# adityaX1412/Experiment-YOLO

Hardware: AMD Instinct MI355X
Metric: images/sec (train) DEAL-YOLO-N 640x640 bs=64/GPU (higher is better)
Workload: dtype f16; 1 GPU; DEAL-YOLO-N (yolov8n-ASF-P2P2.yaml) train step 640x640, per-GPU batch 64, fwd+TAL/WIOU+NWD/DFL/BCE loss+bwd+SGD+EMA, BASELINE.json configs[1]; loss_mode=wiou+nwd, settle_steps=18, capture_retries=0, global_batch=64, parallelism=dp1, hipgraph=True

## Files before the change

experiment-yolo_amd/csrc/bn_act.hip:

```cpp
#include <cstdlib>
#include "common.h"
#include "dealyolo_hip.h"

struct BnFinArgs {
  const float* part[3];
  int nparts[3];
  float pweight[3];
  const float* gamma;
  const float* beta;
  float* running_mean;
  float* running_var;
  float* coef;
  int C;
  float count, eps, momentum;
  int update_running;
  int ldp;
  long long* nbt;
};

__global__ __launch_bounds__(256) void bn_finalize_kernel(BnFinArgs a) {
  const int c = blockIdx.x, tid = threadIdx.x;
  double s1 = 0.0, s2 = 0.0;
  for (int k = 0; k < 3; ++k) {
    if (!a.part[k]) continue;
    double t1 = 0.0, t2 = 0.0;
    for (int i = tid; i < a.nparts[k]; i += 256) {
      t1 += a.part[k][((size_t)i * 2 + 0) * a.ldp + c];
      t2 += a.part[k][((size_t)i * 2 + 1) * a.ldp + c];
    }
    s1 += t1 * a.pweight[k];
    s2 += t2 * a.pweight[k];
  }
  __shared__ double r1[256], r2[256];
  r1[tid] = s1;
  r2[tid] = s2;
  __syncthreads();
  for (int o = 128; o > 0; o >>= 1) {
    if (tid < o) {
      r1[tid] += r1[tid + o];
      r2[tid] += r2[tid + o];
    }
    __syncthreads();
  }
  if (tid == 0) {
    const double mean = r1[0] / a.count;
    double var = r2[0] / a.count - mean * mean;
    if (var < 0.0) var = 0.0;
    const float invstd = (float)(1.0 / sqrt(var + (double)a.eps));
    const float sc = a.gamma[c] * invstd;
    a.coef[0 * a.C + c] = sc;
    a.coef[1 * a.C + c] = a.beta[c] - (float)mean * sc;
    a.coef[2 * a.C + c] = (float)mean;
    a.coef[3 * a.C + c] = invstd;
    if (a.update_running) {
      const double unbiased = a.count > 1.f ? var * a.count / (a.count - 1.0) : var;
      a.running_mean[c] = (1.f - a.momentum) * a.running_mean[c] + a.momentum * (float)mean;
      a.running_var[c] = (1.f - a.momentum) * a.running_var[c] + a.momentum * (float)unbiased;
      if (a.nbt && c == 0) *a.nbt += 1;
    }
  }
}

extern "C" int dy_bn_finalize(const float* p0, int n0, float w0, const float* p1, int n1, float w1, const float* p2,
                              int n2, float w2, const float* gamma, const float* beta, float* running_mean,
                              float* running_var, float* coef, int C, float count, float eps, float momentum,
                              int update_running, hipStream_t stream) {
  BnFinArgs a{{p0, p1, p2}, {n0, n1, n2}, {w0, w1, w2}, gamma, beta, running_mean, running_var, coef, C, count, eps,
              momentum, update_running, C, nullptr};
  hipLaunchKernelGGL(bn_finalize_kernel, dim3(C), dim3(256), 0, stream, a);
  DY_CHECK_LAUNCH();
  return DY_OK;
}
extern "C" int dy_bn_finalize_ld(const float* part, int nparts, int ldp, const float* gamma, const float* beta, float* running_mean,
                                 float* running_var, float* coef, int C, float count, float eps, float momentum, int update_running,
                                 long long* num_batches_tracked, hipStream_t stream) {
  if (C < 1 || ldp < C || nparts < 1 || !part || !gamma || !beta || !coef || (update_running && (!running_mean || !running_var))) return DY_ERR_ARG;
  BnFinArgs a{{part, nullptr, nullptr}, {nparts, 0, 0}, {1.f, 0.f, 0.f}, gamma, beta, running_mean, running_var, coef, C, count, eps,
              momentum, update_running, ldp, update_running ? num_batches_tracked : nullptr};
  hipLaunchKernelGGL(bn_finalize_kernel, dim3(C), dim3(256), 0, stream, a);
  DY_CHECK_LAUNCH();
  return DY_OK;
}

__global__ void bn_eval_coef_kernel(const float* g, const float* b, const float* rm, const float* rv, float* coef, int C,
                                    float eps) {
  const int c = blockIdx.x * blockDim.x + threadIdx.x;
  if (c >= C) return;
  const float invstd = 1.f / sqrtf(rv[c] + eps), sc = g[c] * invstd;
  coef[c] = sc;
  coef[C + c] = b[c] - rm[c] * sc;
  coef[2 * C + c] = rm[c];
  coef[3 * C + c] = invstd;
}
extern "C" int dy_bn_eval_coef(const float* gamma, const float* beta, const float* rm, const float* rv, float* coef,
                               int C, float eps, hipStream_t stream) {
  hipLaunchKernelGGL(bn_eval_coef_kernel, dim3(cdiv(C, 64)), dim3(64), 0, stream, gamma, beta, rm, rv, coef, C, eps);
  DY_CHECK_LAUNCH();
  return DY_OK;
}

#define DY_ACT_DISPATCH(KERNEL, grid, stream, args)                                                        \
  do {                                                                                                     \
    if (act == DY_ACT_SILU) hipLaunchKernelGGL(KERNEL<DY_ACT_SILU>, grid, dim3(256), 0, stream, args);      \
    else if (act == DY_ACT_LEAKY) hipLaunchKernelGGL(KERNEL<DY_ACT_LEAKY>, grid, dim3(256), 0, stream, args); \
    else hipLaunchKernelGGL(KERNEL<DY_ACT_NONE>, grid, dim3(256), 0, stream, args);                         \
  } while (0)

static __device__ __forceinline__ float act_fwd(float z, int act) {
  if (act == DY_ACT_SILU) return silu_f(z);
  if (act == DY_ACT_LEAKY) return z > 0.f ? z : 0.1f * z;
  return z;
}
static __device__ __forceinline__ float act_grad(float z, int act) {
  if (act == DY_ACT_SILU) {
    const float s = sigmoid_f(z);
    return s * (1.f + z * (1.f - s));
  }
  if (act == DY_ACT_LEAKY) return z > 0.f ? 1.f : 0.1f;
  return 1.f;
}

struct ApplyArgs {
  const f16* x;
  const f16* res;
  f16* y;
  const float* coef;
  int ldx, ldr, ldy, C, act;
  long npix;
  int rev;
  f16* y2 = nullptr;
  int ldy2 = 0, csplit = 1 << 30;
};

struct BnAccFwd {
  const double* acc;
  const float* gamma;
  const float* beta;
  float* running_mean;
  float* running_var;
  float* coef_out;
  float count, eps, momentum;
};

template <int ACT, bool ACC, bool FAST = false>
static __device__ __forceinline__ void bn_act_apply_body(const ApplyArgs& a, const BnAccFwd& b, const int bx, const int nb) {
  const int cpp = a.C >> 3, rows = 256 / cpp;
  const int part = threadIdx.x % cpp, row = threadIdx.x / cpp, c0 = part * 8;
  extern __shared__ float s_coef[];
  if (ACC) {
    for (int c = threadIdx.x; c < a.C; c += 256) {
      double s1 = 0.0, s2 = 0.0;
#pragma unroll
      for (int k = 0; k < DY_BN_COPIES; ++k) {
        s1 += b.acc[(size_t)(k * 2 + 0) * a.C + c];
        s2 += b.acc[(size_t)(k * 2 + 1) * a.C + c];
      }
      const double mean = s1 / b.count;
      double var = s2 / b.count - mean * mean;
      if (var < 0.0) var = 0.0;
      const float invstd = (float)(1.0 / sqrt(var + (double)b.eps));
      const float scl = b.gamma[c] * invstd, shf = b.beta[c] - (float)mean * scl;
      s_coef[c] = scl;
      s_coef[a.C + c] = shf;
      if (bx == 0) {
        b.coef_out[c] = scl;
        b.coef_out[a.C + c] = shf;
        b.coef_out[2 * a.C + c] = (float)mean;
        b.coef_out[3 * a.C + c] = invstd;
        const double unbiased = b.count > 1.f ? var * b.count / (b.count - 1.0) : var;
        b.running_mean[c] = (1.f - b.momentum) * b.running_mean[c] + b.momentum * (float)mean;
        b.running_var[c] = (1.f - b.momentum) * b.running_var[c] + b.momentum * (float)unbiased;
      }
    }
    __syncthreads();
  }
  if (row >= rows) return;
  float sc[8], sh[8];
#pragma unroll
  for (int j = 0; j < 8; ++j) {
    sc[j] = ACC ? s_coef[c0 + j] : a.coef[c0 + j];
    sh[j] = ACC ? s_coef[a.C + c0 + j] : a.coef[a.C + c0 + j];
  }
  auto at = [&](long p) { return a.rev ? a.npix - 1 - p : p; };
  f16* const yb = c0 < a.csplit ? a.y + c0 : a.y2 + (c0 - a.csplit);
  const int ly = c0 < a.csplit ? a.ldy : a.ldy2;
  auto one = [&](long pix, const half8& xv) {
    pix = at(pix);
    half8 rv;
    if (a.res) rv = *reinterpret_cast<const half8*>(a.res + pix * a.ldr + c0);
    half8 out;
    if (FAST) {
#pragma unroll
      for (int j = 0; j < 8; j += 2) {
        f32x2 z = act_fwd2_fast<ACT>(__builtin_elementwise_fma((f32x2){(float)xv[j], (float)xv[j + 1]}, (f32x2){sc[j], sc[j + 1]},
                                                               (f32x2){sh[j], sh[j + 1]}));
        if (a.res) z += (f32x2){(float)rv[j], (float)rv[j + 1]};
        const half2_ oh = __builtin_convertvector(z, half2_);
        out[j] = oh[0];
        out[j + 1] = oh[1];
      }
    } else {
#pragma unroll
      for (int j = 0; j < 8; ++j) {
        float z = act_fwd_t<ACT>((float)xv[j] * sc[j] + sh[j]);
        if (a.res) z += (float)rv[j];
        out[j] = (f16)z;
      }
    }
    *reinterpret_cast<half8*>(yb + pix * ly) = out;
  };
  const long step = (long)nb * rows;
  long pix = (long)bx * rows + row;
  for (; pix + step < a.npix; pix += 2 * step) {
    const half8 x0 = *reinterpret_cast<const half8*>(a.x + at(pix) * a.ldx + c0);
    const half8 x1 = *reinterpret_cast<const half8*>(a.x + at(pix + step) * a.ldx + c0);
    one(pix, x0);
    one(pix + step, x1);
  }
  if (pix < a.npix) one(pix, *reinterpret_cast<const half8*>(a.x + at(pix) * a.ldx + c0));
}

template <int ACT, bool ACC, bool FAST = false>
__global__ __launch_bounds__(256) void bn_act_apply_kernel(ApplyArgs a, BnAccFwd b) {
  bn_act_apply_body<ACT, ACC, FAST>(a, b, (int)blockIdx.x, (int)gridDim.x);
}
#define DY_BN_GROUP_MAX 8
struct ApplyGroup {
  int n;
  int nblk[DY_BN_GROUP_MAX];
  ApplyArgs a[DY_BN_GROUP_MAX];
  BnAccFwd b[DY_BN_GROUP_MAX];
};
__global__ __launch_bounds__(256) void bn_act_apply_group_kernel(ApplyGroup g) {
  const int e = blockIdx.y;
  if ((int)blockIdx.x >= g.nblk[e]) return;
  bn_act_apply_body<DY_ACT_SILU, true, true>(g.a[e], g.b[e], (int)blockIdx.x, g.nblk[e]);
}

static inline int ew_reverse() {
  static const int rev = getenv("DY_EW_REVERSE") ? atoi(getenv("DY_EW_REVERSE")) : 4;
  return rev;
}

static long ew_cap(const char* env, long dflt) {
  static struct { const char* name; long cap; } seen[8];
  static int n = 0;
  for (int i = 0; i < n; ++i)
    if (seen[i].name == env) return seen[i].cap;
  const char* e = getenv(env);
  const long cap = e ? atol(e) : dflt;
  if (n < 8) seen[n++] = {env, cap};
  return cap;
}
static inline int ew_blocks(long npix, int C, const char* env, long dflt) {
  const int rows = 256 / (C >> 3);
  long blocks = (npix + (long)rows * 4 - 1) / ((long)rows * 4);
  const long cap = ew_cap(env, dflt);
  if (blocks > cap) blocks = cap;
  if (blocks < 1) blocks = 1;
  return (int)blocks;
}

extern "C" int dy_bn_act_apply(const void* x, int ldx, const void* res, int ldr, void* y, int ldy, const float* coef,
                               long npix, int C, int act, hipStream_t stream) {
  if ((C & 7) || (ldx & 7) || (ldy & 7) || (res && (ldr & 7))) return DY_ERR_ALIGN;
  if ((C >> 3) > 256) return DY_ERR_ARG;
  const int rev = ew_reverse();
  ApplyArgs a{(const f16*)x, (const f16*)res, (f16*)y, coef, ldx, ldr, ldy, C, act, npix, rev & 1};
  const BnAccFwd b{};
  const dim3 grid(ew_blocks(npix, C, "DY_EW_BLOCKS_APPLY", 8192));
  if (act == DY_ACT_SILU) hipLaunchKernelGGL((bn_act_apply_kernel<DY_ACT_SILU, false>), grid, dim3(256), 0, stream, a, b);
  else if (act == DY_ACT_LEAKY) hipLaunchKernelGGL((bn_act_apply_kernel<DY_ACT_LEAKY, false>), grid, dim3(256), 0, stream, a, b);
  else hipLaunchKernelGGL((bn_act_apply_kernel<DY_ACT_NONE, false>), grid, dim3(256), 0, stream, a, b);
  DY_CHECK_LAUNCH();
  return DY_OK;
}

extern "C" int dy_bn_act_apply_acc(const void* x, int ldx, const void* res, int ldr, void* y, int ldy, const double* acc,
                                   const float* gamma, const float* beta, float* running_mean, float* running_var,
                                   float* coef, long npix, int C, int act, float count, float eps, float momentum,
                                   hipStream_t stream) {
  if ((C & 7) || (ldx & 7) || (ldy & 7) || (res && (ldr & 7))) return DY_ERR_ALIGN;
  if ((C >> 3) > 256 || !acc || !gamma || !beta || !running_mean || !running_var || !coef) return DY_ERR_ARG;
  const int rev = ew_reverse();
  ApplyArgs a{(const f16*)x, (const f16*)res, (f16*)y, nullptr, ldx, ldr, ldy, C, act, npix, rev & 1};
  const BnAccFwd b{acc, gamma, beta, running_mean, running_var, coef, count, eps, momentum};
  const dim3 grid(ew_blocks(npix, C, "DY_EW_BLOCKS_APPLY_ACC", 8192));
  const size_t lds = 2 * (size_t)C * sizeof(float);
  static const bool fast = !getenv("DY_SILU_FAST") || atoi(getenv("DY_SILU_FAST"));
  if (act == DY_ACT_SILU && fast) hipLaunchKernelGGL((bn_act_apply_kernel<DY_ACT_SILU, true, true>), grid, dim3(256), lds, stream, a, b);
  else if (act == DY_ACT_SILU) hipLaunchKernelGGL((bn_act_apply_kernel<DY_ACT_SILU, true>), grid, dim3(256), lds, stream, a, b);
  else if (act == DY_ACT_LEAKY) hipLaunchKernelGGL((bn_act_apply_kernel<DY_ACT_LEAKY, true>), grid, dim3(256), lds, stream, a, b);
  else hipLaunchKernelGGL((bn_act_apply_kernel<DY_ACT_NONE, true>), grid, dim3(256), lds, stream, a, b);
  DY_CHECK_LAUNCH();
  return DY_OK;
}

extern "C" int dy_bn_act_apply_acc_split(const void* x, int ldx, void* y, int ldy, void* y2, int ldy2, int csplit, const double* acc,
                                         const float* gamma, const float* beta, float* running_mean, float* running_var, float* coef,
                                         long npix, int C, int act, float count, float eps, float momentum, hipStream_t stream) {
  if ((C & 7) || (ldx & 7) || (ldy & 7) || (ldy2 & 7) || (csplit & 7) || csplit <= 0 || csplit >= C || !y2) return DY_ERR_ALIGN;
  if ((C >> 3) > 256 || !acc || !gamma || !beta || !running_mean || !running_var || !coef) return DY_ERR_ARG;
  const int rev = ew_reverse();
  ApplyArgs a{(const f16*)x, nullptr, (f16*)y, nullptr, ldx, 0, ldy, C, act, npix, rev & 1};
  a.y2 = (f16*)y2; a.ldy2 = ldy2; a.csplit = csplit;
  const BnAccFwd b{acc, gamma, beta, running_mean, running_var, coef, count, eps, momentum};
  const dim3 grid(ew_blocks(npix, C, "DY_EW_BLOCKS_APPLY_ACC", 8192));
  const size_t lds = 2 * (size_t)C * sizeof(float);
  if (act == DY_ACT_SILU) hipLaunchKernelGGL((bn_act_apply_kernel<DY_ACT_SILU, true, true>), grid, dim3(256), lds, stream, a, b);
  else if (act == DY_ACT_LEAKY) hipLaunchKernelGGL((bn_act_apply_kernel<DY_ACT_LEAKY, true>), grid, dim3(256), lds, stream, a, b);
  else hipLaunchKernelGGL((bn_act_apply_kernel<DY_ACT_NONE, true>), grid, dim3(256), lds, stream, a, b);
  DY_CHECK_LAUNCH();
  return DY_OK;
}

extern "C" int dy_bn_group_max(void) { return DY_BN_GROUP_MAX; }
extern "C" int dy_bn_act_apply_acc_group(int n, const void* const* x, const int* ldx, void* const* y, const int* ldy, const double* const* acc,
                                         const float* const* gamma, const float* const* beta, float* const* running_mean,
                                         float* const* running_var, float* const* coef, const long* npix, const int* C, const float* count,
                                         const float* eps, const float* momentum, hipStream_t stream) {
  if (n < 1 || n > DY_BN_GROUP_MAX) return DY_ERR_ARG;
  ApplyGroup g{};
  g.n = n;
  int gx = 1, cmax = 0;
  const int rev = ew_reverse();
  for (int e = 0; e < n; ++e) {
    if ((C[e] & 7) || (ldx[e] & 7) || (ldy[e] & 7)) return DY_ERR_ALIGN;
    if ((C[e] >> 3) > 256 || !acc[e] || !gamma[e] || !beta[e] || !running_mean[e] || !running_var[e] || !coef[e]) return DY_ERR_ARG;
    g.a[e] = ApplyArgs{(const f16*)x[e], nullptr, (f16*)y[e], nullptr, ldx[e], 0, ldy[e], C[e], DY_ACT_SILU, npix[e], rev & 1};
    g.b[e] = BnAccFwd{acc[e], gamma[e], beta[e], running_mean[e], running_var[e], coef[e], count[e], eps[e], momentum[e]};
    g.nblk[e] = ew_blocks(npix[e], C[e], "DY_EW_BLOCKS_APPLY_ACC", 8192);
    gx = g.nblk[e] > gx ? g.nblk[e] : gx;
    cmax = C[e] > cmax ? C[e] : cmax;
  }
  hipLaunchKernelGGL(bn_act_apply_group_kernel, dim3(gx, n), dim3(256), 2 * (size_t)cmax * sizeof(float), stream, g);
  DY_CHECK_LAUNCH();
  return DY_OK;
}

struct BwdRedArgs {
  const f16* dy;
  const f16* x;
  const float* coef;
  float* partials;
  int lddy, ldx, C, act;
  long npix;
  int rev;
  double* acc;
  f16* rg;
  int ldrg, rg_acc;
  const f16* dy2 = nullptr;
  int lddy2 = 0, csplit = 1 << 30;
};

template <int ACT, bool RES = false>
static __device__ __forceinline__ void bn_act_bwd_reduce_body(const BwdRedArgs& a, const int bx, const int nb) {
  const int cpp = a.C >> 3, rows = 256 / cpp, tid = threadIdx.x;
  const int part = tid % cpp, row = tid / cpp, c0 = part * 8;
  f32x2 sg[4], sgx[4], sc[4], sh[4];
#pragma unroll
  for (int j = 0; j < 4; ++j) {
    sg[j] = sgx[j] = (f32x2){0.f, 0.f};
    sc[j] = (f32x2){a.coef[c0 + 2 * j], a.coef[c0 + 2 * j + 1]};
    sh[j] = (f32x2){a.coef[a.C + c0 + 2 * j], a.coef[a.C + c0 + 2 * j + 1]};
  }
  if (row < rows) {
    const long step = (long)nb * rows;
    long pix = (long)bx * rows + row;
    auto at = [&](long p) { return a.rev ? a.npix - 1 - p : p; };
    const f16* const dyb = c0 < a.csplit ? a.dy + c0 : a.dy2 + (c0 - a.csplit);
    const int ldd = c0 < a.csplit ? a.lddy : a.lddy2;
    auto pair = [](const half8& v, int j) { return (f32x2){(float)v[2 * j], (float)v[2 * j + 1]}; };
    auto pass_on = [&](long p, const half8& dv) {
      f16* dst = a.rg + at(p) * a.ldrg + c0;
      half8 o = dv;
      if (a.rg_acc) {
        const half8 old = *reinterpret_cast<const half8*>(dst);
#pragma unroll
        for (int j = 0; j < 8; ++j) o[j] = (f16)((float)old[j] + (float)dv[j]);
      }
      *reinterpret_cast<half8*>(dst) = o;
    };
    for (; pix + step < a.npix; pix += 2 * step) {
      const half8 dv0 = *reinterpret_cast<const half8*>(dyb + at(pix) * ldd);
      const half8 xv0 = *reinterpret_cast<const half8*>(a.x + at(pix) * a.ldx + c0);
      const half8 dv1 = *reinterpret_cast<const half8*>(dyb + at(pix + step) * ldd);
      const half8 xv1 = *reinterpret_cast<const half8*>(a.x + at(pix + step) * a.ldx + c0);
      if (RES) {
        pass_on(pix, dv0);
        pass_on(pix + step, dv1);
      }
#pragma unroll
      for (int j = 0; j < 4; ++j) {
        const f32x2 x0 = pair(xv0, j), x1 = pair(xv1, j);
        const f32x2 g0 = pair(dv0, j) * act_grad2<ACT>(__builtin_elementwise_fma(x0, sc[j], sh[j]));
        const f32x2 g1 = pair(dv1, j) * act_grad2<ACT>(__builtin_elementwise_fma(x1, sc[j], sh[j]));
        sg[j] += g0 + g1;
        sgx[j] += __builtin_elementwise_fma(g0, x0, g1 * x1);
      }
    }
    if (pix < a.npix) {
      const half8 dv = *reinterpret_cast<const half8*>(dyb + at(pix) * ldd);
      const half8 xv = *reinterpret_cast<const half8*>(a.x + at(pix) * a.ldx + c0);
      if (RES) pass_on(pix, dv);
#pragma unroll
      for (int j = 0; j < 4; ++j) {
        const f32x2 x = pair(xv, j);
        const f32x2 g = pair(dv, j) * act_grad2<ACT>(__builtin_elementwise_fma(x, sc[j], sh[j]));
        sg[j] += g;
        sgx[j] += g * x;
      }
    }
#pragma unroll
    for (int j = 0; j < 4; ++j)
#pragma unroll
      for (int k = 0; k < 2; ++k)
        sgx[j][k] = (sgx[j][k] - a.coef[2 * a.C + c0 + 2 * j + k] * sg[j][k]) * a.coef[3 * a.C + c0 + 2 * j + k];
  }
  __shared__ float red[2][256][8 + 1];
#pragma unroll
  for (int j = 0; j < 8; ++j) {
    red[0][tid][j] = sg[j >> 1][j & 1];
    red[1][tid][j] = sgx[j >> 1][j & 1];
  }
  __syncthreads();
  for (int i = tid; i < 2 * a.C; i += 256) {
    const int which = i / a.C, c = i - which * a.C, pp = c >> 3, j = c & 7;
    float s = 0.f;
    for (int r = 0; r < rows; ++r) s += red[which][r * cpp + pp][j];
    if (a.acc) unsafeAtomicAdd(&a.acc[((size_t)(bx % DY_BN_COPIES) * 2 + which) * a.C + c], (double)s);
    else a.partials[((size_t)bx * 2 + which) * a.C + c] = s;
  }
}

template <int ACT, bool RES = false>
__global__ __launch_bounds__(256) void bn_act_bwd_reduce_kernel(BwdRedArgs a) {
  bn_act_bwd_reduce_body<ACT, RES>(a, (int)blockIdx.x, (int)gridDim.x);
}
struct BwdRedGroup {
  int n;
  int nblk[DY_BN_GROUP_MAX];
  BwdRedArgs a[DY_BN_GROUP_MAX];
};
__global__ __launch_bounds__(256) void bn_act_bwd_reduce_group_kernel(BwdRedGroup g) {
  const int e = blockIdx.y;
  if ((int)blockIdx.x >= g.nblk[e]) return;
  bn_act_bwd_reduce_body<DY_ACT_SILU, false>(g.a[e], (int)blockIdx.x, g.nblk[e]);
}

extern "C" int dy_bn_act_bwd_reduce(const void* dy, int lddy, const void* x, int ldx, const float* coef,
                                    float* partials, int max_partials, long npix, int C, int act, int* nparts,
                                    hipStream_t stream) {
  if ((C & 7) || C > 2048 || (ldx & 7) || (lddy & 7)) return DY_ERR_ALIGN;
  const int cpp = C >> 3;
  if (cpp > 256) return DY_ERR_ARG;
  const int rows = 256 / cpp;
  long blocks = (npix + (long)rows * 8 - 1) / ((long)rows * 8);
  if (blocks > max_partials) blocks = max_partials;
  static const long bcap = getenv("DY_EW_BLOCKS_BRED") ? atol(getenv("DY_EW_BLOCKS_BRED")) : 1024;
  if (blocks > bcap) blocks = bcap;
  if (blocks < 1) blocks = 1;
  if (nparts) *nparts = (int)blocks;
  const int rev = ew_reverse();
  BwdRedArgs a{(const f16*)dy, (const f16*)x, coef, partials, lddy, ldx, C, act, npix, (rev >> 2) & 1, nullptr, nullptr, 0, 0};
  DY_ACT_DISPATCH(bn_act_bwd_reduce_kernel, dim3((int)blocks), stream, a);
  DY_CHECK_LAUNCH();
  return DY_OK;
}

extern "C" int dy_bn_act_bwd_reduce_acc(const void* dy, int lddy, const void* x, int ldx, const float* coef, double* acc,
                                        long npix, int C, int act, void* res_grad, int ldrg, int res_accumulate, hipStream_t stream) {
  if ((C & 7) || C > 2048 || (ldx & 7) || (lddy & 7) || (res_grad && ((ldrg & 7) || ((uintptr_t)res_grad & 15)))) return DY_ERR_ALIGN;
  const int cpp = C >> 3;
  if (cpp > 256 || !acc) return DY_ERR_ARG;
  const int rows = 256 / cpp;
  long blocks = (npix + (long)rows * 8 - 1) / ((long)rows * 8);
  static const long bcap = getenv("DY_EW_BLOCKS_BRED") ? atol(getenv("DY_EW_BLOCKS_BRED")) : 1024;
  if (blocks > bcap) blocks = bcap;
  if (blocks < 1) blocks = 1;
  const int rev = ew_reverse();
  BwdRedArgs a{(const f16*)dy, (const f16*)x, coef, nullptr, lddy, ldx, C, act, npix, (rev >> 2) & 1, acc, (f16*)res_grad, ldrg, res_accumulate};
  if (res_grad && act == DY_ACT_SILU) hipLaunchKernelGGL((bn_act_bwd_reduce_kernel<DY_ACT_SILU, true>), dim3((int)blocks), dim3(256), 0, stream, a);
  else if (res_grad && act == DY_ACT_LEAKY) hipLaunchKernelGGL((bn_act_bwd_reduce_kernel<DY_ACT_LEAKY, true>), dim3((int)blocks), dim3(256), 0, stream, a);
  else if (res_grad) hipLaunchKernelGGL((bn_act_bwd_reduce_kernel<DY_ACT_NONE, true>), dim3((int)blocks), dim3(256), 0, stream, a);
  else DY_ACT_DISPATCH(bn_act_bwd_reduce_kernel, dim3((int)blocks), stream, a);
  DY_CHECK_LAUNCH();
  return DY_OK;
}

extern "C" int dy_bn_act_bwd_reduce_acc_split(const void* dy, int lddy, const void* dy2, int lddy2, int csplit, const void* x, int ldx,
                                              const float* coef, double* acc, long npix, int C, int act, hipStream_t stream) {
  if ((C & 7) || C > 2048 || (ldx & 7) || (lddy & 7) || (lddy2 & 7) || (csplit & 7) || csplit <= 0 || csplit >= C || !dy2) return DY_ERR_ALIGN;
  const int cpp = C >> 3;
  if (cpp > 256 || !acc) return DY_ERR_ARG;
  const int rows = 256 / cpp;
  long blocks = (npix + (long)rows * 8 - 1) / ((long)rows * 8);
  static const long bcap = getenv("DY_EW_BLOCKS_BRED") ? atol(getenv("DY_EW_BLOCKS_BRED")) : 1024;
  if (blocks > bcap) blocks = bcap;
  if (blocks < 1) blocks = 1;
  const int rev = ew_reverse();
  BwdRedArgs a{(const f16*)dy, (const f16*)x, coef, nullptr, lddy, ldx, C, act, npix, (rev >> 2) & 1, acc, nullptr, 0, 0};
  a.dy2 = (const f16*)dy2; a.lddy2 = lddy2; a.csplit = csplit;
  DY_ACT_DISPATCH(bn_act_bwd_reduce_kernel, dim3((int)blocks), stream, a);
  DY_CHECK_LAUNCH();
  return DY_OK;
}

extern "C" int dy_bn_act_bwd_reduce_acc_group(int n, const void* const* dy, const int* lddy, const void* const* x, const int* ldx,
                                              const float* const* coef, double* const* acc, const long* npix, const int* C, hipStream_t stream) {
  if (n < 1 || n > DY_BN_GROUP_MAX) return DY_ERR_ARG;
  BwdRedGroup g{};
  g.n = n;
  int gx = 1;
  const int rev = ew_reverse();
  static const long bcap = getenv("DY_EW_BLOCKS_BRED") ? atol(getenv("DY_EW_BLOCKS_BRED")) : 1024;
  for (int e = 0; e < n; ++e) {
    if ((C[e] & 7) || C[e] > 2048 || (ldx[e] & 7) || (lddy[e] & 7)) return DY_ERR_ALIGN;
    const int cpp = C[e] >> 3;
    if (cpp > 256 || !acc[e] || !dy[e] || !x[e] || !coef[e]) return DY_ERR_ARG;
    const int rows = 256 / cpp;
    long blocks = (npix[e] + (long)rows * 8 - 1) / ((long)rows * 8);
    if (blocks > bcap) blocks = bcap;
    if (blocks < 1) blocks = 1;
    g.a[e] = BwdRedArgs{(const f16*)dy[e], (const f16*)x[e], coef[e], nullptr, lddy[e], ldx[e], C[e], DY_ACT_SILU, npix[e], (rev >> 2) & 1, acc[e],
                        nullptr, 0, 0};
    g.nblk[e] = (int)blocks;
    gx = g.nblk[e] > gx ? g.nblk[e] : gx;
  }
  hipLaunchKernelGGL(bn_act_bwd_reduce_group_kernel, dim3(gx, n), dim3(256), 0, stream, g);
  DY_CHECK_LAUNCH();
  return DY_OK;
}

struct BwdRedRowsArgs {
  const f16* dy;
  const f16* x;
  const float* coef;
  double* acc;
  const int* flag;
  int lddy, ldx, C, A, a0, hw, B;
};
template <int ACT>
__global__ __launch_bounds__(256) void bn_act_bwd_reduce_rows_kernel(BwdRedRowsArgs a) {
  __shared__ int s_list[256];
  __shared__ int s_cnt[4];
  __shared__ float red[2][256][8 + 1];
  const int cpp = a.C >> 3, rows = 256 / cpp, tid = threadIdx.x, wave = tid >> 6, lane = tid & 63;
  const int part = tid % cpp, row = tid / cpp, c0 = part * 8;
  f32x2 sg[4], sgx[4], sc[4], sh[4];
#pragma unroll
  for (int j = 0; j < 4; ++j) {
    sg[j] = sgx[j] = (f32x2){0.f, 0.f};
    sc[j] = (f32x2){a.coef[c0 + 2 * j], a.coef[c0 + 2 * j + 1]};
    sh[j] = (f32x2){a.coef[a.C + c0 + 2 * j], a.coef[a.C + c0 + 2 * j + 1]};
  }
  const long npix = (long)a.B * a.hw;
  const long chunk = (npix + gridDim.x - 1) / gridDim.x;
  const long lo = (long)blockIdx.x * chunk, hi = lo + chunk < npix ? lo + chunk : npix;
  constexpr int FB = 8;
  int fl[FB];
  for (long p0 = lo, trip = 0; p0 < hi; p0 += 256, ++trip) {
    if ((trip & (FB - 1)) == 0) {
#pragma unroll
      for (int k = 0; k < FB; ++k) {
        const long pk = p0 + (long)k * 256 + tid;
        fl[k] = -1;
        if (pk < hi) {
          const int b = (int)(pk / a.hw), r = (int)(pk - (long)b * a.hw);
          fl[k] = a.flag[(size_t)b * a.A + a.a0 + r];
        }
      }
    }
    int mine = -1;
#pragma unroll
    for (int k = 0; k < FB; ++k)
      if ((trip & (FB - 1)) == k) mine = fl[k];
    const bool fg = mine >= 0;
    const unsigned long long m = __ballot(fg);
    if (lane == 0) s_cnt[wave] = __popcll(m);
    __syncthreads();
    int base = 0, total = 0;
#pragma unroll
    for (int w = 0; w < 4; ++w) {
      if (w < wave) base += s_cnt[w];
      total += s_cnt[w];
    }
    if (fg) s_list[base + __popcll(m & ((1ull << lane) - 1ull))] = tid;
    __syncthreads();
    if (row < rows) {
      for (int i = row; i < total; i += rows) {
        const long q = p0 + s_list[i];
        const half8 dv = *reinterpret_cast<const half8*>(a.dy + q * a.lddy + c0);
        const half8 xv = *reinterpret_cast<const half8*>(a.x + q * a.ldx + c0);
#pragma unroll
        for (int j = 0; j < 4; ++j) {
          const f32x2 x = (f32x2){(float)xv[2 * j], (float)xv[2 * j + 1]};
          const f32x2 g = (f32x2){(float)dv[2 * j], (float)dv[2 * j + 1]} * act_grad2<ACT>(__builtin_elementwise_fma(x, sc[j], sh[j]));
          sg[j] += g;
          sgx[j] += g * x;
        }
      }
    }
    __syncthreads();
  }
#pragma unroll
  for (int j = 0; j < 4; ++j)
#pragma unroll
    for (int k = 0; k < 2; ++k)
      sgx[j][k] = (sgx[j][k] - a.coef[2 * a.C + c0 + 2 * j + k] * sg[j][k]) * a.coef[3 * a.C + c0 + 2 * j + k];
#pragma unroll
  for (int j = 0; j < 8; ++j) {
    red[0][tid][j] = row < rows ? sg[j >> 1][j & 1] : 0.f;
    red[1][tid][j] = row < rows ? sgx[j >> 1][j & 1] : 0.f;
  }
  __syncthreads();
  for (int i = tid; i < 2 * a.C; i += 256) {
    const int which = i / a.C, c = i - which * a.C, pp = c >> 3, j = c & 7;
    float t = 0.f;
    for (int r = 0; r < rows; ++r) t += red[which][r * cpp + pp][j];
    if (t != 0.f) unsafeAtomicAdd(&a.acc[((size_t)(blockIdx.x % DY_BN_COPIES) * 2 + which) * a.C + c], (double)t);
  }
}
extern "C" int dy_bn_act_bwd_reduce_rows(const void* dy, int lddy, const void* x, int ldx, const float* coef, double* acc, int n,
                                         int hw, int C, int act, const int* assigned, int A, int a0, hipStream_t stream) {
  if ((C & 7) || (ldx & 7) || (lddy & 7)) return DY_ERR_ALIGN;
  const int cpp = C >> 3;
  if (cpp > 256 || !acc || !assigned || n < 1 || hw < 1 || a0 < 0 || a0 + hw > A) return DY_ERR_ARG;
  BwdRedRowsArgs a{(const f16*)dy, (const f16*)x, coef, acc, assigned, lddy, ldx, C, A, a0, hw, n};
  DY_ACT_DISPATCH(bn_act_bwd_reduce_rows_kernel, dim3(1024), stream, a);
  DY_CHECK_LAUNCH();
  return DY_OK;
}

__global__ __launch_bounds__(256) void bn_bwd_finalize_kernel(const float* partials, int nparts, float* dgamma,
                                                              float* dbeta, float* bwdcoef, int C, float count,
                                                              int accumulate, int ldp) {
  const int c = blockIdx.x, tid = threadIdx.x;
  double s1 = 0.0, s2 = 0.0;
// ... 349 lines not shown
```

Before: 6190 images/s.

## Prefetch BN-apply inputs ahead of coefficient reduction and deepen per-thread load batching

Rewrites the fused BN+activation apply kernel so each thread issues a batch of four pixel loads (and residual loads) before the per-channel statistic finalisation and barrier, overlapping global-memory latency with the reduction. It specialises the kernel on whether a residual is present, uses pointer-stride iteration instead of per-pixel index math, and adds an occupancy hint to the launch bounds. The grid is resized to cover eight pixels per thread and rounded to a multiple of 256 CUs, falling back to the old sizing for small tensors. The old path stays available behind an environment flag; the costs are extra register pressure from the load buffers and fewer blocks.

Result: no change. 6224 images/s, median of 6 (+0.5%).

```diff
diff --git a/experiment-yolo_amd/csrc/bn_act.hip b/experiment-yolo_amd/csrc/bn_act.hip
--- a/experiment-yolo_amd/csrc/bn_act.hip
+++ b/experiment-yolo_amd/csrc/bn_act.hip
@@ -142,18 +142,71 @@
   float count, eps, momentum;
 };
 
-template <int ACT, bool ACC, bool FAST = false>
+static inline bool bn_v1() {
+  const char* e = getenv("DY_BN_V1");
+  return e && e[0] == '1' && !e[1];
+}
+
+#ifndef DY_BN_APPLY_DEPTH
+#define DY_BN_APPLY_DEPTH 4
+#endif
+#ifndef DY_BN_APPLY_WAVES
+#define DY_BN_APPLY_WAVES 4
+#endif
+template <int ACT, bool ACC, bool FAST, bool RESID>
 static __device__ __forceinline__ void bn_act_apply_body(const ApplyArgs& a, const BnAccFwd& b, const int bx, const int nb) {
+  constexpr int U = DY_BN_APPLY_DEPTH;
   const int cpp = a.C >> 3, rows = 256 / cpp;
   const int part = threadIdx.x % cpp, row = threadIdx.x / cpp, c0 = part * 8;
+  const long step = (long)nb * rows, pix0 = (long)bx * rows + row;
+  const long n = row < rows && pix0 < a.npix ? (a.npix - pix0 + step - 1) / step : 0;
+  const long first = a.rev ? a.npix - 1 - pix0 : pix0, dir = a.rev ? -step : step;
   extern __shared__ float s_coef[];
+  double p1[DY_BN_COPIES], p2[DY_BN_COPIES];
+  if (ACC && (int)threadIdx.x < a.C) {
+#pragma unroll
+    for (int k = 0; k < DY_BN_COPIES; ++k) {
+      p1[k] = b.acc[(size_t)(k * 2 + 0) * a.C + threadIdx.x];
+      p2[k] = b.acc[(size_t)(k * 2 + 1) * a.C + threadIdx.x];
+    }
+  }
+  half8 xv[U] = {}, rv[U] = {};
+  const f16* px = a.x + first * a.ldx + c0;
+  const f16* pr = RESID ? a.res + first * a.ldr + c0 : nullptr;
+  const long sx = dir * a.ldx, sr = RESID ? dir * a.ldr : 0;
+  auto fetch = [&](half8& x, half8& r) {
+    x = *reinterpret_cast<const half8*>(px);
+    px += sx;
+    if (RESID) {
+      r = *reinterpret_cast<const half8*>(pr);
+      pr += sr;
+    }
+  };
+  auto fetch_round = [&](long k) {
+    if (k + U <= n) {
+#pragma unroll
+      for (int u = 0; u < U; ++u) fetch(xv[u], rv[u]);
+    } else {
+#pragma unroll
+      for (int u = 0; u < U; ++u)
+        if (k + u < n) fetch(xv[u], rv[u]);
+    }
+  };
+  fetch_round(0);
   if (ACC) {
     for (int c = threadIdx.x; c < a.C; c += 256) {
+      if (c != (int)threadIdx.x) {
+#pragma unroll
+        for (int k = 0; k < DY_BN_COPIES; ++k) {
+          p1[k] = b.acc[(size_t)(k * 2 + 0) * a.C + c];
+          p2[k] = b.acc[(size_t)(k * 2 + 1) * a.C + c];
+        }
+      }
       double s1 = 0.0, s2 = 0.0;
 #pragma unroll
       for (int k = 0; k < DY_BN_COPIES; ++k) {
-        s1 += b.acc[(size_t)(k * 2 + 0) * a.C + c];
-        s2 += b.acc[(size_t)(k * 2 + 1) * a.C + c];
+        s1 += p1[k];
+        s2 += p2[k];
       }
       const double mean = s1 / b.count;
       double var = s2 / b.count - mean * mean;
@@ -174,6 +227,88 @@
     }
     __syncthreads();
   }
+  if (n == 0) return;
+  float sc[8], sh[8];
+#pragma unroll
+  for (int j = 0; j < 8; ++j) {
+    sc[j] = ACC ? s_coef[c0 + j] : a.coef[c0 + j];
+    sh[j] = ACC ? s_coef[a.C + c0 + j] : a.coef[a.C + c0 + j];
+  }
+  f16* const yb = c0 < a.csplit ? a.y + c0 : a.y2 + (c0 - a.csplit);
+  const int ly = c0 < a.csplit ? a.ldy : a.ldy2;
+  f16* py = yb + first * ly;
+  const long sy = dir * ly;
+  auto one = [&](const half8& x, const half8& r) {
+    half8 out;
+    if (FAST) {
+#pragma unroll
+      for (int j = 0; j < 8; j += 2) {
+        f32x2 z = act_fwd2_fast<ACT>(__builtin_elementwise_fma((f32x2){(float)x[j], (float)x[j + 1]}, (f32x2){sc[j], sc[j + 1]},
+                                                               (f32x2){sh[j], sh[j + 1]}));
+        if (RESID) z += (f32x2){(float)r[j], (float)r[j + 1]};
+        const half2_ oh = __builtin_convertvector(z, half2_);
+        out[j] = oh[0];
+        out[j + 1] = oh[1];
+      }
+    } else {
+#pragma unroll
+      for (int j = 0; j < 8; ++j) {
+        float z = act_fwd_t<ACT>((float)x[j] * sc[j] + sh[j]);
+        if (RESID) z += (float)r[j];
+        out[j] = (f16)z;
+      }
+    }
+    *reinterpret_cast<half8*>(py) = out;
+    py += sy;
+  };
+#pragma unroll 1
+  for (long k = 0;;) {
+    if (k + U <= n) {
+#pragma unroll
+      for (int u = 0; u < U; ++u) one(xv[u], rv[u]);
+    } else {
+#pragma unroll
+      for (int u = 0; u < U; ++u)
+        if (k + u < n) one(xv[u], rv[u]);
+    }
+    k += U;
+    if (k >= n) break;
+    fetch_round(k);
+  }
+}
+
+template <int ACT, bool ACC, bool FAST = false>
+static __device__ __forceinline__ void bn_act_apply_body_v1(const ApplyArgs& a, const BnAccFwd& b, const int bx, const int nb) {
+  const int cpp = a.C >> 3, rows = 256 / cpp;
+  const int part = threadIdx.x % cpp, row = threadIdx.x / cpp, c0 = part * 8;
+  extern __shared__ float s_coef[];
+  if (ACC) {
+    for (int c = threadIdx.x; c < a.C; c += 256) {
+      double s1 = 0.0, s2 = 0.0;
+#pragma unroll
+      for (int k = 0; k < DY_BN_COPIES; ++k) {
+        s1 += b.acc[(size_t)(k * 2 + 0) * a.C + c];
+        s2 += b.acc[(size_t)(k * 2 + 1) * a.C + c];
+      }
+      const double mean = s1 / b.count;
+      double var = s2 / b.count - mean * mean;
+      if (var < 0.0) var = 0.0;
+      const float invstd = (float)(1.0 / sqrt(var + (double)b.eps));
+      const float scl = b.gamma[c] * invstd, shf = b.beta[c] - (float)mean * scl;
+      s_coef[c] = scl;
+      s_coef[a.C + c] = shf;
+      if (bx == 0) {
+        b.coef_out[c] = scl;
+        b.coef_out[a.C + c] = shf;
+        b.coef_out[2 * a.C + c] = (float)mean;
+        b.coef_out[3 * a.C + c] = invstd;
+        const double unbiased = b.count > 1.f ? var * b.count / (b.count - 1.0) : var;
+        b.running_mean[c] = (1.f - b.momentum) * b.running_mean[c] + b.momentum * (float)mean;
+        b.running_var[c] = (1.f - b.momentum) * b.running_var[c] + b.momentum * (float)unbiased;
+      }
+    }
+    __syncthreads();
+  }
   if (row >= rows) return;
   float sc[8], sh[8];
 #pragma unroll
@@ -221,8 +356,13 @@
 }
 
 template <int ACT, bool ACC, bool FAST = false>
-__global__ __launch_bounds__(256) void bn_act_apply_kernel(ApplyArgs a, BnAccFwd b) {
-  bn_act_apply_body<ACT, ACC, FAST>(a, b, (int)blockIdx.x, (int)gridDim.x);
+__global__ __launch_bounds__(256, DY_BN_APPLY_WAVES) void bn_act_apply_kernel(ApplyArgs a, BnAccFwd b) {
+  if (a.res) bn_act_apply_body<ACT, ACC, FAST, true>(a, b, (int)blockIdx.x, (int)gridDim.x);
+  else bn_act_apply_body<ACT, ACC, FAST, false>(a, b, (int)blockIdx.x, (int)gridDim.x);
+}
+template <int ACT, bool ACC, bool FAST = false>
+__global__ __launch_bounds__(256) void bn_act_apply_v1_kernel(ApplyArgs a, BnAccFwd b) {
+  bn_act_apply_body_v1<ACT, ACC, FAST>(a, b, (int)blockIdx.x, (int)gridDim.x);
 }
 #define DY_BN_GROUP_MAX 8
 struct ApplyGroup {
@@ -231,10 +371,15 @@
   ApplyArgs a[DY_BN_GROUP_MAX];
   BnAccFwd b[DY_BN_GROUP_MAX];
 };
-__global__ __launch_bounds__(256) void bn_act_apply_group_kernel(ApplyGroup g) {
+__global__ __launch_bounds__(256, DY_BN_APPLY_WAVES) void bn_act_apply_group_kernel(ApplyGroup g) {
   const int e = blockIdx.y;
   if ((int)blockIdx.x >= g.nblk[e]) return;
-  bn_act_apply_body<DY_ACT_SILU, true, true>(g.a[e], g.b[e], (int)blockIdx.x, g.nblk[e]);
+  bn_act_apply_body<DY_ACT_SILU, true, true, false>(g.a[e], g.b[e], (int)blockIdx.x, g.nblk[e]);
+}
+__global__ __launch_bounds__(256) void bn_act_apply_group_v1_kernel(ApplyGroup g) {
+  const int e = blockIdx.y;
+  if ((int)blockIdx.x >= g.nblk[e]) return;
+  bn_act_apply_body_v1<DY_ACT_SILU, true, true>(g.a[e], g.b[e], (int)blockIdx.x, g.nblk[e]);
 }
 
 static inline int ew_reverse() {
@@ -260,6 +405,25 @@
   if (blocks < 1) blocks = 1;
   return (int)blocks;
 }
+#ifndef DY_BN_APPLY_PPT
+#define DY_BN_APPLY_PPT 8
+#endif
+#define DY_BN_CUS 256
+static inline int apply_blocks(long npix, int C, const char* env, long dflt, bool v1) {
+  if (v1) return ew_blocks(npix, C, env, dflt);
+  const int rows = 256 / (C >> 3);
+  long blocks = (npix + (long)rows * DY_BN_APPLY_PPT - 1) / ((long)rows * DY_BN_APPLY_PPT);
+  const long cap = ew_cap(env, dflt);
+  if (blocks > cap) blocks = cap;
+  blocks -= blocks % DY_BN_CUS;
+  if (blocks < 3 * DY_BN_CUS) return ew_blocks(npix, C, env, dflt);
+  return (int)blocks;
+}
+#define DY_APPLY_LAUNCH(v1, grid, lds, stream, a, b, ...)                                                          \
+  do {                                                                                                             \
+    if (v1) hipLaunchKernelGGL((bn_act_apply_v1_kernel<__VA_ARGS__>), grid, dim3(256), lds, stream, a, b);        \
+    else hipLaunchKernelGGL((bn_act_apply_kernel<__VA_ARGS__>), grid, dim3(256), lds, stream, a, b);               \
+  } while (0)
 
 extern "C" int dy_bn_act_apply(const void* x, int ldx, const void* res, int ldr, void* y, int ldy, const float* coef,
                                long npix, int C, int act, hipStream_t stream) {
@@ -268,10 +432,11 @@
   const int rev = ew_reverse();
   ApplyArgs a{(const f16*)x, (const f16*)res, (f16*)y, coef, ldx, ldr, ldy, C, act, npix, rev & 1};
   const BnAccFwd b{};
-  const dim3 grid(ew_blocks(npix, C, "DY_EW_BLOCKS_APPLY", 8192));
-  if (act == DY_ACT_SILU) hipLaunchKernelGGL((bn_act_apply_kernel<DY_ACT_SILU, false>), grid, dim3(256), 0, stream, a, b);
-  else if (act == DY_ACT_LEAKY) hipLaunchKernelGGL((bn_act_apply_kernel<DY_ACT_LEAKY, false>), grid, dim3(256), 0, stream, a, b);
-  else hipLaunchKernelGGL((bn_act_apply_kernel<DY_ACT_NONE, false>), grid, dim3(256), 0, stream, a, b);
+  const bool v1 = bn_v1();
+  const dim3 grid(apply_blocks(npix, C, "DY_EW_BLOCKS_APPLY", 8192, v1));
+  if (act == DY_ACT_SILU) DY_APPLY_LAUNCH(v1, grid, 0, stream, a, b, DY_ACT_SILU, false);
+  else if (act == DY_ACT_LEAKY) DY_APPLY_LAUNCH(v1, grid, 0, stream, a, b, DY_ACT_LEAKY, false);
+  else DY_APPLY_LAUNCH(v1, grid, 0, stream, a, b, DY_ACT_NONE, false);
   DY_CHECK_LAUNCH();
   return DY_OK;
 }
@@ -285,13 +450,14 @@
   const int rev = ew_reverse();
   ApplyArgs a{(const f16*)x, (const f16*)res, (f16*)y, nullptr, ldx, ldr, ldy, C, act, npix, rev & 1};
   const BnAccFwd b{acc, gamma, beta, running_mean, running_var, coef, count, eps, momentum};
-  const dim3 grid(ew_blocks(npix, C, "DY_EW_BLOCKS_APPLY_ACC", 8192));
+  const bool v1 = bn_v1();
+  const dim3 grid(apply_blocks(npix, C, "DY_EW_BLOCKS_APPLY_ACC", 8192, v1));
   const size_t lds = 2 * (size_t)C * sizeof(float);
   static const bool fast = !getenv("DY_SILU_FAST") || atoi(getenv("DY_SILU_FAST"));
-  if (act == DY_ACT_SILU && fast) hipLaunchKernelGGL((bn_act_apply_kernel<DY_ACT_SILU, true, true>), grid, dim3(256), lds, stream, a, b);
-  else if (act == DY_ACT_SILU) hipLaunchKernelGGL((bn_act_apply_kernel<DY_ACT_SILU, true>), grid, dim3(256), lds, stream, a, b);
-  else if (act == DY_ACT_LEAKY) hipLaunchKernelGGL((bn_act_apply_kernel<DY_ACT_LEAKY, true>), grid, dim3(256), lds, stream, a, b);
-  else hipLaunchKernelGGL((bn_act_apply_kernel<DY_ACT_NONE, true>), grid, dim3(256), lds, stream, a, b);
+  if (act == DY_ACT_SILU && fast) DY_APPLY_LAUNCH(v1, grid, lds, stream, a, b, DY_ACT_SILU, true, true);
+  else if (act == DY_ACT_SILU) DY_APPLY_LAUNCH(v1, grid, lds, stream, a, b, DY_ACT_SILU, true);
+  else if (act == DY_ACT_LEAKY) DY_APPLY_LAUNCH(v1, grid, lds, stream, a, b, DY_ACT_LEAKY, true);
+  else DY_APPLY_LAUNCH(v1, grid, lds, stream, a, b, DY_ACT_NONE, true);
   DY_CHECK_LAUNCH();
   return DY_OK;
 }
@@ -305,11 +471,12 @@
   ApplyArgs a{(const f16*)x, nullptr, (f16*)y, nullptr, ldx, 0, ldy, C, act, npix, rev & 1};
   a.y2 = (f16*)y2; a.ldy2 = ldy2; a.csplit = csplit;
   const BnAccFwd b{acc, gamma, beta, running_mean, running_var, coef, count, eps, momentum};
-  const dim3 grid(ew_blocks(npix, C, "DY_EW_BLOCKS_APPLY_ACC", 8192));
+  const bool v1 = bn_v1();
+  const dim3 grid(apply_blocks(npix, C, "DY_EW_BLOCKS_APPLY_ACC", 8192, v1));
   const size_t lds = 2 * (size_t)C * sizeof(float);
-  if (act == DY_ACT_SILU) hipLaunchKernelGGL((bn_act_apply_kernel<DY_ACT_SILU, true, true>), grid, dim3(256), lds, stream, a, b);
-  else if (act == DY_ACT_LEAKY) hipLaunchKernelGGL((bn_act_apply_kernel<DY_ACT_LEAKY, true>), grid, dim3(256), lds, stream, a, b);
-  else hipLaunchKernelGGL((bn_act_apply_kernel<DY_ACT_NONE, true>), grid, dim3(256), lds, stream, a, b);
+  if (act == DY_ACT_SILU) DY_APPLY_LAUNCH(v1, grid, lds, stream, a, b, DY_ACT_SILU, true, true);
+  else if (act == DY_ACT_LEAKY) DY_APPLY_LAUNCH(v1, grid, lds, stream, a, b, DY_ACT_LEAKY, true);
+  else DY_APPLY_LAUNCH(v1, grid, lds, stream, a, b, DY_ACT_NONE, true);
   DY_CHECK_LAUNCH();
   return DY_OK;
 }
@@ -324,16 +491,17 @@
   g.n = n;
   int gx = 1, cmax = 0;
   const int rev = ew_reverse();
+  const bool v1 = bn_v1();
   for (int e = 0; e < n; ++e) {
     if ((C[e] & 7) || (ldx[e] & 7) || (ldy[e] & 7)) return DY_ERR_ALIGN;
     if ((C[e] >> 3) > 256 || !acc[e] || !gamma[e] || !beta[e] || !running_mean[e] || !running_var[e] || !coef[e]) return DY_ERR_ARG;
     g.a[e] = ApplyArgs{(const f16*)x[e], nullptr, (f16*)y[e], nullptr, ldx[e], 0, ldy[e], C[e], DY_ACT_SILU, npix[e], rev & 1};
     g.b[e] = BnAccFwd{acc[e], gamma[e], beta[e], running_mean[e], running_var[e], coef[e], count[e], eps[e], momentum[e]};
-    g.nblk[e] = ew_blocks(npix[e], C[e], "DY_EW_BLOCKS_APPLY_ACC", 8192);
+    g.nblk[e] = apply_blocks(npix[e], C[e], "DY_EW_BLOCKS_APPLY_ACC", 8192, v1);
     gx = g.nblk[e] > gx ? g.nblk[e] : gx;
     cmax = C[e] > cmax ? C[e] : cmax;
   }
-  hipLaunchKernelGGL(bn_act_apply_group_kernel, dim3(gx, n), dim3(256), 2 * (size_t)cmax * sizeof(float), stream, g);
+  hipLaunchKernelGGL(v1 ? bn_act_apply_group_v1_kernel : bn_act_apply_group_kernel, dim3(gx, n), dim3(256), 2 * (size_t)cmax * sizeof(float), stream, g);
   DY_CHECK_LAUNCH();
   return DY_OK;
 }
```
